# lipku/LiveTalking

Hardware: NVIDIA H100
Metric: lip-sync frames/sec (wav2lip256, 256x256, batch 16, mel + U-Net fwd + paste-back) (higher is better)
Workload: dtype f16 (fp32 accumulate); mel f64; paste u8

## Files before the change

### livetalking_b200/csrc/conv_halo.cu

```cuda
#include <cuda.h>

#include <atomic>
#include <mutex>
#include <utility>

#include "conv_halo.h"
#include "ltb_internal.h"
#include "ptx_sm90.cuh"

#ifdef LTB_HALO_DIAG
#include <cstdlib>
#define LTB_DIAG(bit) (p.dbg & (bit))
#else
#define LTB_DIAG(bit) 0
#endif

namespace ltb {

constexpr int kHaloP = 10;
constexpr int kHaloThreads = 384;
constexpr int kProducerRegs = 40, kConsumerRegs = 232;
constexpr int kSms = 132;

template <int BN, int NSUB, int NACC, int TAPS, int RC = 0>
struct HaloCfg {
  static constexpr bool HALO = (TAPS != 1);
  static constexpr bool S2 = (TAPS == 10);
  static constexpr int P = S2 ? 9 : (HALO ? kHaloP : 8);
  static constexpr int HR = S2 ? 16 * NSUB + 1 : (HALO ? 16 * NSUB + 2 : 16 * NSUB);
  static constexpr int TG = (TAPS == 9 || TAPS == 10) ? 3 : (TAPS == 16 ? 4 : 1);
  static constexpr int PLANE_BYTES = (HR * P * 128 + 1023) & ~1023;
  static constexpr int A_BYTES_RAW = (S2 ? 4 : 1) * HR * P * 128;
  static constexpr int A_BYTES = S2 ? 4 * PLANE_BYTES : ((A_BYTES_RAW + 1023) & ~1023);
  static constexpr int B_BYTES = TG * BN * 128;
  static constexpr int BUDGET = 223 * 1024;
  static constexpr int A_STAGES_STREAM = S2 ? 2 : ((BN <= 32) ? 4 : (BN <= 64 ? 3 : (NSUB == 1 ? 3 : 2)));
  static constexpr int A_STAGES_RES = ((BUDGET - RC * TG * B_BYTES) / A_BYTES) > 4 ? 4 : ((BUDGET - RC * TG * B_BYTES) / A_BYTES);
  static constexpr int A_STAGES = RC ? A_STAGES_RES : A_STAGES_STREAM;
  static constexpr bool RES_PREFETCH = (BN == 128 && NSUB == 2 && NACC == 1 && TAPS == 9 && RC == 0);
  static constexpr int RES_BYTES = RES_PREFETCH ? 128 * BN * 2 : 0;
  static constexpr int B_STAGES_MAX = (BUDGET - A_STAGES * A_BYTES - RES_BYTES) / B_BYTES;
  static constexpr int B_STAGES = RC ? RC * TG : (B_STAGES_MAX > 8 ? 8 : B_STAGES_MAX);
  static constexpr bool LAG = RC || B_STAGES >= 2 * TG;
  static constexpr int ACOLS = NACC * BN;
  static constexpr int SMEM_BYTES = A_STAGES * A_BYTES + B_STAGES * B_BYTES + RES_BYTES + 1024;
  static_assert(NSUB * ACOLS <= 256, "register accumulator overflow");
  static_assert(B_STAGES >= 2, "not enough shared memory for the weight ring");
  static_assert(A_STAGES >= 2, "not enough shared memory for the halo ring");
  static_assert(SMEM_BYTES + 3584 <= 227 * 1024, "shared memory overflow (dynamic + static)");
};

struct SubpixelView {
  int stage, view, slot0, brow, nslots;
};
constexpr int subpixel_view(int vy, int vx) { return (vy + 1) * kHaloP + (vx + 1); }
template <int TAPS>
struct SubpixelTable;
template <>
struct SubpixelTable<9> {
  static constexpr int NV = 5;
  static constexpr SubpixelView v[NV] = {{0, 0, 0, 0, 3}, {1, 1, 1, 0, 2}, {1, kHaloP + 1, 2, 2, 1}, {2, 0, 3, 2, 1}, {2, kHaloP, 2, 0, 2}};
};
template <>
struct SubpixelTable<16> {
  static constexpr int NV = 10;
  static constexpr SubpixelView v[NV] = {{0, subpixel_view(0, 0), 0, 0, 4},
                                         {1, subpixel_view(-1, 0), 0, 0, 2},  {1, subpixel_view(0, 1), 1, 2, 2},
                                         {2, subpixel_view(1, 0), 2, 0, 2},   {2, subpixel_view(0, -1), 0, 2, 1}, {2, subpixel_view(0, -1), 3, 3, 1},
                                         {3, subpixel_view(-1, -1), 0, 0, 1}, {3, subpixel_view(-1, 1), 1, 1, 1}, {3, subpixel_view(1, 1), 2, 2, 1},
                                         {3, subpixel_view(1, -1), 3, 3, 1}};
};

template <int BN, int SLOT0, int BROW, int R, size_t... S>
__device__ __forceinline__ void subpixel_slots(float (&acc)[R], uint64_t a, uint32_t b_lo, uint32_t b_hi, std::index_sequence<S...>) {
  (wgmma_ss_at<BN, (SLOT0 + (int)S) * BN>(acc, a, wgmma_lohi(b_lo + (BROW + (uint32_t)S) * BN * 8u, b_hi), 1u), ...);
}

template <int BN, int TAPS, int R, size_t... V>
__device__ __forceinline__ void subpixel_issue(float (&acc)[R], int j, int k, uint32_t a_lo0, uint32_t b_lo0, uint32_t a_hi, uint32_t b_hi,
                                               std::index_sequence<V...>) {
  (
      [&] {
        constexpr SubpixelView g = SubpixelTable<TAPS>::v[V];
        if (j == g.stage)
          subpixel_slots<BN, g.slot0, g.brow>(acc, wgmma_lohi(a_lo0 + g.view * 8u + k * 2u, a_hi), b_lo0 + k * 2u, b_hi,
                                              std::make_index_sequence<g.nslots>{});
      }(),
      ...);
}

__device__ __forceinline__ void quad_transpose(uint32_t (&x)[4], int lane) {
  const bool b2 = lane & 2, b1 = lane & 1;
  uint32_t s0 = __shfl_xor_sync(0xffffffffu, b2 ? x[0] : x[2], 2);
  uint32_t s1 = __shfl_xor_sync(0xffffffffu, b2 ? x[1] : x[3], 2);
  x[0] = b2 ? s0 : x[0];
  x[1] = b2 ? s1 : x[1];
  x[2] = b2 ? x[2] : s0;
  x[3] = b2 ? x[3] : s1;
  s0 = __shfl_xor_sync(0xffffffffu, b1 ? x[0] : x[1], 1);
  s1 = __shfl_xor_sync(0xffffffffu, b1 ? x[2] : x[3], 1);
  x[0] = b1 ? s0 : x[0];
  x[2] = b1 ? s1 : x[2];
  x[1] = b1 ? x[1] : s0;
  x[3] = b1 ? x[3] : s1;
}

constexpr bool halo_res_smem_ok(int BN, int NSUB, int NACC, int TAPS) { return TAPS == 9 && NACC == 1 && BN * NSUB <= 128; }

template <int BN, int NSUB, int NACC, int TAPS, int RC, bool GRP>
__global__ void __launch_bounds__(kHaloThreads, 1) conv_halo_wgmma_kernel(const __grid_constant__ HaloParams p) {
  static_assert(!GRP || TAPS == 1, "grouped weights exist in GEMM mode only");
  using C = HaloCfg<BN, NSUB, NACC, TAPS, RC>;
  extern __shared__ uint8_t smem_raw[];
  __shared__ __align__(8) uint64_t a_full[C::A_STAGES], a_empty[C::A_STAGES];
  __shared__ __align__(8) uint64_t b_full[C::B_STAGES], b_empty[C::B_STAGES];
  __shared__ float head_sw[100];
  constexpr int kGnSmem = (NACC == 1) ? 512 : 1;
  __shared__ float gn_acc[kGnSmem];

  const int tid = threadIdx.x, warp = tid >> 5, lane = tid & 31;
  constexpr bool kHeadOk = (BN == 32 && NACC == 1 && TAPS == 9);
  const bool gn_smem = NACC == 1 && p.gn_stats != nullptr && p.gn_images * p.gn_groups * 2 <= kGnSmem;
  if (gn_smem)
    for (int i = tid; i < p.gn_images * p.gn_groups * 2; i += kHaloThreads) gn_acc[i] = 0.f;
  constexpr bool kHaloMode = C::HALO;
  if (kHeadOk && p.head_out && tid < 99) head_sw[tid] = (tid < 96) ? p.head_w[tid] : p.head_b[tid - 96];
  const uint32_t smem0 = (smem_u32(smem_raw) + 1023u) & ~1023u;
  const uint32_t a_smem = smem0;
  const uint32_t b_smem = smem0 + C::A_STAGES * C::A_BYTES;
  const int chunks = (p.Cin + 63) / 64;
  const int kl_last = (p.Cin - 64 * (chunks - 1) + 15) / 16;

  if (tid == 0) {
    for (int s = 0; s < C::A_STAGES; ++s) {
      mbar_init(smem_u32(&a_full[s]), 1);
      mbar_init(smem_u32(&a_empty[s]), 8);
    }
    for (int s = 0; s < C::B_STAGES; ++s) {
      mbar_init(smem_u32(&b_full[s]), 1);
      mbar_init(smem_u32(&b_empty[s]), 8);
    }
    mbar_fence_init();
    tma_prefetch_desc(&p.tm_in);
    tma_prefetch_desc(&p.tm_w);
  }
  __syncthreads();

  const int tiles_m = kHaloMode ? p.tiles_x * p.tiles_y * p.N : p.tiles_x;

  pdl_launch_dependents();
  if (RC && warp == 8 && lane == 0) {
    mbar_arrive_expect_tx(smem_u32(&b_full[0]), RC * C::TG * C::B_BYTES);
    for (int c = 0; c < RC; ++c)
      for (int j = 0; j < C::TG; ++j)
        tma_load_3d(b_smem + (c * C::TG + j) * C::B_BYTES, &p.tm_w, smem_u32(&b_full[0]), c * 64, 0, j * C::TG);
  }
  pdl_wait();

// ... 744 lines not shown
```

### livetalking_b200/csrc/conv_plan.cu

```cuda
#include <cstring>
#include <string>
#include <vector>

#include "../../include/ltb200.h"
#include "conv_plan.h"
#include "ltb_internal.h"

namespace ltb {

static const int kTd[2][2] = {{0, 0}, {0, 1}};
static const int kTk[2][2] = {{1, 0}, {2, 0}};
static const int kTn[2] = {1, 2};
static const int kUd[2][2] = {{-1, 0}, {0, 1}};

ConvParams conv_params(ConvMode mode, int N, ConvSlice in, int IH, int IW, int Cin, ConvSlice out, int OH, int OW, int Cout,
                       ConvSlice res, const __half* w, int Ktot, int w_koff, const float* bias, bool relu, ConvTaps taps) {
  ConvParams p;
  std::memset(&p, 0, sizeof(p));
  p.in = in.p;
  p.N = N;
  p.IH = IH;
  p.IW = IW;
  p.ICtot = in.Ctot;
  p.ic_off = in.off;
// ... 10 lines not shown
  p.RCtot = res.Ctot;
  p.rc_off = res.off;
  p.w = w;
  p.Ktot = Ktot;
  p.bias = bias;
  p.relu = relu ? 1 : 0;
  if (mode == ConvMode::Dense) {
    p.sy = taps.sy;
    p.sx = taps.sx;
    p.GH = OH;
    p.GW = OW;
    p.nphases = 1;
    ConvPhase& ph = p.ph[0];
    ph.ntaps = taps.KH * taps.KW;
    ph.koff = w_koff;
    for (int kh = 0; kh < taps.KH; ++kh)
      for (int kw = 0; kw < taps.KW; ++kw) {
        ph.dy[kh * taps.KW + kw] = (signed char)(kh - taps.pad_t);
        ph.dx[kh * taps.KW + kw] = (signed char)(kw - taps.pad_l);
      }
  } else {
    const bool up = mode == ConvMode::Upsample2x;
    p.GH = IH;
    p.GW = IW;
    p.osy = p.osx = 2;
    p.nphases = 4;
    p.upconv = up ? 1 : 0;
    int koff = w_koff;
    for (int a = 0; a < 2; ++a)
      for (int b = 0; b < 2; ++b) {
        ConvPhase& ph = p.ph[a * 2 + b];
        const int na = up ? 2 : kTn[a], nb = up ? 2 : kTn[b];
        ph.ntaps = na * nb;
        ph.koff = koff;
        ph.ooy = a;
        ph.oox = b;
        for (int i = 0; i < na; ++i)
          for (int j = 0; j < nb; ++j) {
            ph.dy[i * nb + j] = (signed char)(up ? kUd[a][i] : kTd[a][i]);
            ph.dx[i * nb + j] = (signed char)(up ? kUd[b][j] : kTd[b][j]);
          }
        koff += ph.ntaps * Cin;
      }
  }
  p.M = N * p.GH * p.GW;
  return p;
}

int conv_plan(const ConvParams& p, const __half* w_tap, ConvPath path, ConvPlan* out) {
  out->p = p;
  out->halo = false;
  out->pingpong = false;
  out->rowpair = false;
  if (p.group_slot) {
    if (p.group_images < 1 || p.N % p.group_images || p.slots < 1 || p.w_slot_stride < 0 || p.bias_slot_stride < 0)
      return LTB_FAIL("conv: grouped weights need N divisible by group_images >= 1, slots >= 1 and non-negative slot strides");
    if (p.zbatch > 1 || p.upconv) return LTB_FAIL("conv: grouped weights cannot be combined with zbatch or the fused upsample");
  }
  if (path == ConvPath::Gather) return 0;
  if (w_tap && conv_pingpong_supported(p)) {
    if (conv_pingpong_make_plan(p, w_tap, &out->pp) != 0) return LTB_FAIL("conv: ping-pong plan / tensor map creation failed");
    out->pingpong = true;
    return 0;
  }
  if (w_tap && conv_rowpair_supported(p)) {
    if (conv_rowpair_make_plan(p, w_tap, &out->rp) != 0) return LTB_FAIL("conv: row-pair plan / tensor map creation failed");
    out->rowpair = true;
    return 0;
  }
  const bool gemm = p.nphases == 1 && p.ph[0].ntaps == 1;
  if (!((w_tap || gemm) && conv_halo_supported(p))) {
    if (path == ConvPath::Auto) return 0;
    return LTB_FAIL("conv: the halo kernel cannot run " + std::to_string(p.N) + "x" + std::to_string(p.IH) + "x" + std::to_string(p.IW) +
                    "x" + std::to_string(p.Cin) + " -> " + std::to_string(p.OH) + "x" + std::to_string(p.OW) + "x" + std::to_string(p.Cout) +
                    (w_tap || gemm ? "" : " without tap-major weights"));
  }
  if (conv_halo_make_plan(p, w_tap, &out->hp) != 0) return LTB_FAIL("conv: halo plan / tensor map creation failed");
  out->halo = true;
  return 0;
}

cudaError_t conv_launch(const ConvPlan& pl, cudaStream_t st, float* splitk_ws, size_t ws_floats) {
  if (pl.pingpong) return launch_conv_pingpong(pl.pp, st);
  if (pl.rowpair) return launch_conv_rowpair(pl.rp, st);
  return pl.halo ? launch_conv_halo(pl.hp, st) : launch_conv_gather(pl.p, st, splitk_ws, ws_floats);
}

bool conv_plan_variant(const ConvPlan& pl, bool have_ws, size_t ws_floats, ltb_conv_variant* out) {
  std::memset(out, 0, sizeof(*out));
  out->grouped = pl.p.group_slot != nullptr;
  if (pl.pingpong) {
    out->kernel = 2;
    out->taps = 9;
    out->bn = 64;
    out->nsub = 1;
    out->nacc = 1;
    out->resident_chunks = 1;
    out->res_halo = 1;
    return true;
  }
  if (pl.rowpair) {
    out->kernel = 3;
    out->taps = 9;
    out->bn = 32;
    out->nsub = 1;
    out->nacc = 1;
    out->resident_chunks = 2;
    return true;
  }
  if (pl.halo) {
    out->kernel = 1;
    out->taps = pl.hp.TAPS;
    out->bn = pl.hp.BN;
    out->nsub = pl.hp.NSUB;
    out->nacc = pl.hp.NACC;
    out->resident_chunks = conv_halo_resident_chunks(pl.hp, conv_halo_sms());
    out->res_halo = pl.hp.hp.res_halo;
    return true;
  }
  int ksplit = 0;
  if (!conv_gather_pick(pl.p, have_ws, ws_floats, &out->bn, &out->kb, &ksplit)) return false;
  out->ksplit = ksplit > 1 ? ksplit : 1;
  return true;
}

bool conv_plan_fuse_gn_stats(ConvPlan* pl, float* stats, int groups, int hw) {
  const ConvParams& p = pl->p;
  if (!pl->halo || pl->hp.grouped || p.oc_off != 0 || p.OCtot != p.Cout || !conv_halo_gn_fusable(pl->hp, p.Cout, groups, hw)) return false;
  HaloParams& h = pl->hp.hp;
  h.gn_stats = stats;
  h.gn_groups = groups;
  h.gn_cpg = p.Cout / groups;
  h.gn_hw = hw;
  h.gn_images = p.M / hw;
  return true;
}

bool conv_plan_fuse_head(ConvPlan* pl, const float* w, const float* b, float* out) {
  if (pl->rowpair) {
    pl->rp.head_w = w;
    pl->rp.head_b = b;
    pl->rp.head_out = out;
    return true;
  }
  if (!pl->halo || pl->hp.grouped || pl->hp.BN != 32 || pl->p.Cout != 32) return false;
  pl->hp.hp.head_w = w;
  pl->hp.hp.head_b = b;
  pl->hp.hp.head_out = out;
  return true;
}

static void pack_conv_w(const float* w, int cout, int cin, int KH, int KW, std::vector<__half>& out) {
  out.resize((size_t)cout * KH * KW * cin);
  for (int co = 0; co < cout; ++co)
    for (int kh = 0; kh < KH; ++kh)
      for (int kw = 0; kw < KW; ++kw)
        for (int ci = 0; ci < cin; ++ci)
          out[((size_t)co * KH * KW + kh * KW + kw) * cin + ci] = __float2half(w[(((size_t)co * cin + ci) * KH + kh) * KW + kw]);
}
static void pack_convT_w(const float* w, int cin, int cout, std::vector<__half>& out) {
// ... 36 lines not shown
  }
  if (OH <= 0 || OW <= 0) return LTB_FAIL("empty output");
  const size_t in_b = (size_t)d->N * d->IH * d->IW * d->Cin * 2, out_b = (size_t)d->N * OH * OW * d->Cout * 2;
  __half *din = nullptr, *dout = nullptr, *dw = nullptr, *dres = nullptr, *dwt = nullptr;
  float* dbias = nullptr;
  float* dws = nullptr;
  cudaEvent_t e0 = nullptr, e1 = nullptr;
  int rc = 0;
  auto cleanup = [&]() {
    cudaFree(din);
    cudaFree(dout);
    cudaFree(dw);
    cudaFree(dres);
    cudaFree(dwt);
    cudaFree(dws);
    cudaFree(dbias);
    if (e0) cudaEventDestroy(e0);
    if (e1) cudaEventDestroy(e1);
  };
#define CK(x)                                                             \
  do {                                                                    \
    cudaError_t _e = (x);                                                 \
    if (_e != cudaSuccess) {                                              \
      rc = LTB_FAIL(std::string(#x) + ": " + cudaGetErrorString(_e));     \
      cleanup();                                                          \
      return rc;                                                          \
    }                                                                     \
  } while (0)
  CK(cudaMalloc(&din, in_b));
  CK(cudaMalloc(&dout, out_b));
  CK(cudaMalloc(&dw, wp.size() * 2));
  CK(cudaMalloc(&dbias, (size_t)d->Cout * 4));
  CK(cudaMemcpy(din, in_f16, in_b, cudaMemcpyHostToDevice));
  CK(cudaMemcpy(dw, wp.data(), wp.size() * 2, cudaMemcpyHostToDevice));
  CK(cudaMemcpy(dbias, bias_f32, (size_t)d->Cout * 4, cudaMemcpyHostToDevice));
  CK(cudaMemset(dout, 0xFF, out_b));
  if (d->has_res) {
    CK(cudaMalloc(&dres, out_b));
    CK(cudaMemcpy(dres, res_f16, out_b, cudaMemcpyHostToDevice));
  }
  if (d->KH == 3 && d->KW == 3) {
    CK(cudaMalloc(&dwt, wp.size() * 2));
    CK(d->transposed ? launch_w_tap_major_convT(dw, dwt, d->Cout, d->Cin, nullptr) : launch_w_tap_major(dw, dwt, d->Cout, d->Cin, nullptr));
  }
  const ConvParams p = conv_params(d->transposed ? ConvMode::Transposed : ConvMode::Dense, d->N, {din, d->Cin, 0}, d->IH, d->IW, d->Cin,
                                   {dout, d->Cout, 0}, OH, OW, d->Cout, d->has_res ? ConvSlice{dres, d->Cout, 0} : ConvSlice{}, dw, Ktot, 0,
                                   dbias, d->relu != 0, {d->KH, d->KW, d->sy, d->sx, d->pad, d->pad});
  const ConvPath path = d->force_path == 1 ? ConvPath::Gather : d->force_path == 2 ? ConvPath::Halo : ConvPath::Auto;
  ConvPlan pl;
  if (conv_plan(p, dwt, path, &pl)) {
    cleanup();
    return 1;
  }
  const size_t ws_floats = (pl.halo || pl.pingpong || pl.rowpair) ? 0 : (size_t)1 << 22;
  if (ws_floats) {
    CK(cudaMalloc(&dws, ws_floats * sizeof(float)));
    CK(cudaMemset(dws, 0, ws_floats * sizeof(float)));
  }
  CK(conv_launch(pl, nullptr, dws, ws_floats));
  if (reps > 0) {
    CK(cudaEventCreate(&e0));
    CK(cudaEventCreate(&e1));
    for (int i = 0; i < 3; ++i) CK(conv_launch(pl, nullptr, dws, ws_floats));
    CK(cudaEventRecord(e0, nullptr));
    for (int i = 0; i < reps; ++i) CK(conv_launch(pl, nullptr, dws, ws_floats));
    CK(cudaEventRecord(e1, nullptr));
    CK(cudaEventSynchronize(e1));
    CK(cudaEventElapsedTime(ms_out, e0, e1));
    *ms_out /= reps;
  }
  CK(cudaDeviceSynchronize());
  CK(cudaMemcpy(out_f16, dout, out_b, cudaMemcpyDeviceToHost));
#undef CK
  cleanup();
  return 0;
}

extern "C" {

int ltb_conv2d_f16(const ltb_conv_desc* d, const void* in_f16, const float* w_f32, const float* bias_f32,
                   const void* res_f16, void* out_f16) {
  return conv2d_f16_impl(d, in_f16, w_f32, bias_f32, res_f16, out_f16, 0, nullptr);
}

int ltb_conv2d_f16_timed(const ltb_conv_desc* d, const void* in_f16, const float* w_f32, const float* bias_f32,
                         const void* res_f16, void* out_f16, int reps, float* ms_per_launch) {
  if (reps < 1 || !ms_per_launch) return LTB_FAIL("conv2d_f16_timed: reps >= 1 and a result pointer are required");
  return conv2d_f16_impl(d, in_f16, w_f32, bias_f32, res_f16, out_f16, reps, ms_per_launch);
}

}
```

### livetalking_b200/csrc/conv_plan.h

```cpp
#pragma once
#include <cuda_runtime.h>

#include "conv_halo.h"
#include "conv_pingpong.h"
#include "conv_rowpair.h"

struct ltb_conv_variant;

namespace ltb {

struct ConvSlice {
  const __half* p;
  int Ctot, off;
};

enum class ConvMode {
  Dense,
  Transposed,
  Upsample2x,
};
struct ConvTaps {
  int KH, KW, sy, sx, pad_t, pad_l;
};

inline int conv_out_dim(int in, int k, int s, int pad) { return (in + 2 * pad - k) / s + 1; }

ConvParams conv_params(ConvMode mode, int N, ConvSlice in, int IH, int IW, int Cin, ConvSlice out, int OH, int OW, int Cout,
                       ConvSlice res, const __half* w, int Ktot, int w_koff, const float* bias, bool relu, ConvTaps taps = {});

enum class ConvPath {
  Auto,
  Gather,
  Halo,
};
struct ConvPlan {
  ConvParams p{};
  bool halo = false;
  HaloPlan hp{};
  bool pingpong = false;
  PingpongParams pp{};
  bool rowpair = false;
  RowpairParams rp{};
};

int conv_plan(const ConvParams& p, const __half* w_tap, ConvPath path, ConvPlan* out);
cudaError_t conv_launch(const ConvPlan& pl, cudaStream_t st, float* splitk_ws, size_t ws_floats);
bool conv_plan_variant(const ConvPlan& pl, bool have_ws, size_t ws_floats, ltb_conv_variant* out);

bool conv_plan_fuse_gn_stats(ConvPlan* pl, float* stats, int groups, int hw);
bool conv_plan_fuse_head(ConvPlan* pl, const float* w, const float* b, float* out);

}
```

### livetalking_b200/csrc/ltb_internal.h

```cpp
#pragma once
#include <cuda_runtime.h>
#include <cuda_fp16.h>
#include <cstdint>
#include <cstdio>
#include <atomic>
#include <cstdlib>
#include <utility>
#include <string>

#include "conv_params.h"

namespace ltb {

void set_error(const std::string& msg);
int fail(const char* file, int line, const std::string& msg);
#define LTB_FAIL(msg) ::ltb::fail(__FILE__, __LINE__, (msg))
#define LTB_CUDA(expr)                                                                         \
  do {                                                                                         \
    cudaError_t _e = (expr);                                                                   \
    if (_e != cudaSuccess) {                                                                   \
      cudaGetLastError();  \
      return LTB_FAIL(std::string(#expr) + ": " + cudaGetErrorString(_e));                     \
    }                                                                                          \
  } while (0)

struct SmemConfigOnce {
  std::atomic<unsigned long long> done{0};
  template <typename K>
  cudaError_t ensure(K kernel, int bytes) {
    int dev = 0;
    cudaError_t e = cudaGetDevice(&dev);
    if (e != cudaSuccess) return e;
    const unsigned long long bit = 1ull << (dev & 63);
    if (done.load(std::memory_order_acquire) & bit) return cudaSuccess;
    e = cudaFuncSetAttribute(kernel, cudaFuncAttributeMaxDynamicSharedMemorySize, bytes);
    if (e == cudaSuccess) done.fetch_or(bit, std::memory_order_release);
    return e;
  }
};

bool pdl_default();
bool pdl_enabled();
void pdl_set_enabled(bool on);

template <typename... KArgs, typename... Args>
inline cudaError_t launch_kernel_pdl(void (*kernel)(KArgs...), dim3 grid, dim3 block, size_t smem, cudaStream_t st, Args&&... args) {
  cudaLaunchConfig_t cfg = {};
  cfg.gridDim = grid;
  cfg.blockDim = block;
  cfg.dynamicSmemBytes = smem;
  cfg.stream = st;
  cudaLaunchAttribute attr[1];
  attr[0].id = cudaLaunchAttributeProgrammaticStreamSerialization;
  attr[0].val.programmaticStreamSerializationAllowed = 1;
  cfg.attrs = attr;
  cfg.numAttrs = pdl_enabled() ? 1 : 0;
  return cudaLaunchKernelEx(&cfg, kernel, std::forward<Args>(args)...);
}

template <typename... KArgs, typename... Args>
inline cudaError_t launch_kernel_plain(void (*kernel)(KArgs...), dim3 grid, dim3 block, size_t smem, cudaStream_t st, Args&&... args) {
  cudaLaunchConfig_t cfg = {};
  cfg.gridDim = grid;
  cfg.blockDim = block;
  cfg.dynamicSmemBytes = smem;
  cfg.stream = st;
  cfg.numAttrs = 0;
  return cudaLaunchKernelEx(&cfg, kernel, std::forward<Args>(args)...);
}

struct SlotDesc {
  const uint8_t* face;
  const uint8_t* frame;
  int y1, y2, x1, x2;
};

cudaError_t launch_conv_gather(const ConvParams& p, cudaStream_t st, float* splitk_ws = nullptr, size_t splitk_ws_floats = 0);
bool conv_gather_pick(const ConvParams& p, bool have_ws, size_t splitk_ws_floats, int* bn, int* kb, int* ksplit);

cudaError_t launch_w2l_prep_faces(const uint8_t* faces, int nfaces, const int* d_index, int B, __half* img_pad, cudaStream_t st,
                                  const SlotDesc* slots = nullptr);
cudaError_t launch_set_int(int* p, int v, cudaStream_t st);
cudaError_t launch_w2l_audio_conv0(const float* mel, const float* w9x32, const float* bias, __half* out, int B, cudaStream_t st);
cudaError_t launch_w2l_head(const __half* x, const float* w3x32, const float* b3, float* pred, int npix, cudaStream_t st);

cudaError_t launch_mel_step(const float* pcm, int nsamp, int B, int stride_left_chunks, int fps, double* scratch_spec,
                            double* scratch_mel, float* out, cudaStream_t st);
size_t mel_scratch_spec_doubles(int nsamp);
size_t mel_scratch_mel_doubles(int nsamp);

cudaError_t launch_w2l_paste(const uint8_t* frames, const int* coords, int nf, int H, int W, const float* pred, int slot0,
                             int index, int explicit_idx, int count, uint8_t* out, cudaStream_t st, const SlotDesc* slots = nullptr);

}
```

### livetalking_b200/csrc/ptx_sm90.cuh

```cuda
#pragma once
#include <cuda_fp16.h>
#include <cstdint>
#include <cstdio>

namespace ltb {

__device__ __forceinline__ uint32_t smem_u32(const void* p) {
  return static_cast<uint32_t>(__cvta_generic_to_shared(p));
}

__device__ __forceinline__ void mbar_init(uint32_t bar, uint32_t count) {
  asm volatile("mbarrier.init.shared::cta.b64 [%0], %1;" ::"r"(bar), "r"(count) : "memory");
}
__device__ __forceinline__ void mbar_fence_init() {
  asm volatile("fence.mbarrier_init.release.cluster;" ::: "memory");
}
__device__ __forceinline__ void mbar_arrive(uint32_t bar) {
  asm volatile("mbarrier.arrive.shared::cta.b64 _, [%0];" ::"r"(bar) : "memory");
}
__device__ __forceinline__ void mbar_arrive_expect_tx(uint32_t bar, uint32_t bytes) {
  asm volatile("mbarrier.arrive.expect_tx.shared::cta.b64 _, [%0], %1;" ::"r"(bar), "r"(bytes) : "memory");
}
__device__ __forceinline__ bool mbar_try_wait(uint32_t bar, uint32_t parity) {
  uint32_t ok;
// ... 10 lines not shown
  if (mbar_try_wait(bar, parity)) return;
  const long long t0 = clock64();
  while (!mbar_try_wait(bar, parity)) {
    if (clock64() - t0 > 8000000000LL) __trap();
  }
}

__device__ __forceinline__ void fence_proxy_async_smem() {
  asm volatile("fence.proxy.async.shared::cta;" ::: "memory");
}

__device__ __forceinline__ void cp_async16(uint32_t dst, const void* src, uint32_t src_bytes) {
  asm volatile("cp.async.cg.shared.global [%0], [%1], 16, %2;" ::"r"(dst), "l"(src), "r"(src_bytes) : "memory");
}
__device__ __forceinline__ void cp_async_commit() { asm volatile("cp.async.commit_group;" ::: "memory"); }
template <int N>
__device__ __forceinline__ void cp_async_wait() {
  asm volatile("cp.async.wait_group %0;" ::"n"(N) : "memory");
}
__device__ __forceinline__ uint4 lds128(uint32_t addr) {
  uint4 v;
  asm volatile("ld.shared.v4.u32 {%0, %1, %2, %3}, [%4];" : "=r"(v.x), "=r"(v.y), "=r"(v.z), "=r"(v.w) : "r"(addr) : "memory");
  return v;
}

__device__ __forceinline__ void tma_prefetch_desc(const void* tmap) {
  asm volatile("prefetch.tensormap [%0];" ::"l"(tmap) : "memory");
}
__device__ __forceinline__ void tma_load_2d(uint32_t dst, const void* tmap, uint32_t bar, int c0, int c1) {
  asm volatile(
      "cp.async.bulk.tensor.2d.shared::cluster.global.mbarrier::complete_tx::bytes [%0], [%1, {%3, %4}], [%2];" ::"r"(dst),
      "l"(tmap), "r"(bar), "r"(c0), "r"(c1)
      : "memory");
}
__device__ __forceinline__ void tma_load_3d(uint32_t dst, const void* tmap, uint32_t bar, int c0, int c1, int c2) {
  asm volatile(
      "cp.async.bulk.tensor.3d.shared::cluster.global.mbarrier::complete_tx::bytes [%0], [%1, {%3, %4, %5}], [%2];" ::"r"(dst),
      "l"(tmap), "r"(bar), "r"(c0), "r"(c1), "r"(c2)
      : "memory");
}
__device__ __forceinline__ void tma_load_4d(uint32_t dst, const void* tmap, uint32_t bar, int c0, int c1, int c2, int c3) {
  asm volatile(
      "cp.async.bulk.tensor.4d.shared::cluster.global.mbarrier::complete_tx::bytes [%0], [%1, {%3, %4, %5, %6}], [%2];" ::"r"(
          dst),
      "l"(tmap), "r"(bar), "r"(c0), "r"(c1), "r"(c2), "r"(c3)
      : "memory");
}
__device__ __forceinline__ void tma_load_5d(uint32_t dst, const void* tmap, uint32_t bar, int c0, int c1, int c2, int c3,
                                            int c4) {
  asm volatile(
      "cp.async.bulk.tensor.5d.shared::cluster.global.mbarrier::complete_tx::bytes [%0], [%1, {%3, %4, %5, %6, %7}], [%2];" ::
          "r"(dst),
      "l"(tmap), "r"(bar), "r"(c0), "r"(c1), "r"(c2), "r"(c3), "r"(c4)
      : "memory");
}

__device__ __forceinline__ void ldmatrix_x4(uint32_t& r0, uint32_t& r1, uint32_t& r2, uint32_t& r3, uint32_t saddr) {
  asm volatile("ldmatrix.sync.aligned.m8n8.x4.shared.b16 {%0, %1, %2, %3}, [%4];"
               : "=r"(r0), "=r"(r1), "=r"(r2), "=r"(r3)
               : "r"(saddr)
               : "memory");
}

__device__ __forceinline__ void ldmatrix_x4_trans(uint32_t& r0, uint32_t& r1, uint32_t& r2, uint32_t& r3, uint32_t saddr) {
  asm volatile("ldmatrix.sync.aligned.m8n8.x4.trans.shared.b16 {%0, %1, %2, %3}, [%4];"
               : "=r"(r0), "=r"(r1), "=r"(r2), "=r"(r3)
               : "r"(saddr)
               : "memory");
}
__device__ __forceinline__ void stmatrix_x4_trans(uint32_t saddr, uint32_t r0, uint32_t r1, uint32_t r2, uint32_t r3) {
  asm volatile("stmatrix.sync.aligned.m8n8.x4.trans.shared.b16 [%0], {%1, %2, %3, %4};" ::"r"(saddr), "r"(r0), "r"(r1), "r"(r2), "r"(r3)
               : "memory");
}

__device__ __forceinline__ void tma_store_4d(const void* tmap, uint32_t src, int c0, int c1, int c2, int c3) {
  asm volatile("cp.async.bulk.tensor.4d.global.shared::cta.bulk_group [%0, {%2, %3, %4, %5}], [%1];" ::"l"(tmap), "r"(src), "r"(c0),
               "r"(c1), "r"(c2), "r"(c3)
               : "memory");
}
__device__ __forceinline__ void bulk_commit() { asm volatile("cp.async.bulk.commit_group;" ::: "memory"); }
template <int N>
__device__ __forceinline__ void bulk_wait_read() {
  asm volatile("cp.async.bulk.wait_group.read %0;" ::"n"(N) : "memory");
}
template <int N>
__device__ __forceinline__ void bulk_wait() {
  asm volatile("cp.async.bulk.wait_group %0;" ::"n"(N) : "memory");
}

__device__ __forceinline__ void named_sync(uint32_t id, uint32_t threads) {
  asm volatile("bar.sync %0, %1;" ::"r"(id), "r"(threads) : "memory");
}
__device__ __forceinline__ void named_arrive(uint32_t id, uint32_t threads) {
  asm volatile("bar.arrive %0, %1;" ::"r"(id), "r"(threads) : "memory");
}

__device__ __forceinline__ uint64_t wgmma_desc(uint32_t saddr, uint32_t lbo_bytes, uint32_t sbo_bytes, uint32_t layout) {
  uint64_t d = 0;
  d |= (uint64_t)((saddr & 0x3FFFF) >> 4);
  d |= (uint64_t)((lbo_bytes >> 4) & 0x3FFF) << 16;
  d |= (uint64_t)((sbo_bytes >> 4) & 0x3FFF) << 32;
  d |= (uint64_t)(layout & 3) << 62;
  return d;
}
__host__ __device__ constexpr uint32_t wgmma_hi_128b(uint32_t sbo_bytes) { return (sbo_bytes >> 4) | (1u << 30); }
__host__ __device__ constexpr uint32_t wgmma_hi_32b(uint32_t sbo_bytes) { return (sbo_bytes >> 4) | (3u << 30); }
// ... 204 lines not shown
```

### livetalking_b200/csrc/w2l_engine.cu

```cuda
#include <cstring>
#include <memory>
#include <mutex>
#include <string>
#include <vector>

#include "../../include/ltb200.h"
#include "conv_plan.h"
#include "ltb_internal.h"
#include "stem_umma.h"

namespace ltb {

static thread_local std::string g_last_error;
void set_error(const std::string& msg) { g_last_error = msg; }

bool pdl_default() {
  static const bool on = [] {
    const char* e = std::getenv("LTB_NO_PDL");
    return !(e && e[0] && e[0] != '0');
  }();
  return on;
}
static thread_local int g_pdl = -1;
bool pdl_enabled() { return g_pdl < 0 ? pdl_default() : g_pdl == 1; }
// ... 240 lines not shown
  const int catS[8] = {512, 512, 512, 256, 128, 64, 32, 16};
  __half* cat[8];
  for (int i = 0; i < 8; ++i) {
    void* p;
    if (dev_alloc(s, (size_t)B * catH[i] * catH[i] * (catD[i] + catS[i]) * 2, &p, true)) return 1;
    cat[i] = static_cast<__half*>(p);
  }
  const size_t tmp_bytes = (size_t)B * 256 * 256 * 64 * 2;
  __half* ring[2] = {nullptr, nullptr};
  int ring_next = 0;
  auto new_tmp = [&](int H, int W, int C, View* v) -> int {
    void* p = nullptr;
    if (keep) {
      if (dev_alloc(s, (size_t)B * H * W * C * 2, &p, true)) return 1;
    } else {
      if (!ring[ring_next]) {
        if (dev_alloc(s, tmp_bytes, &p, true)) return 1;
        ring[ring_next] = static_cast<__half*>(p);
      }
      p = ring[ring_next];
      ring_next ^= 1;
    }
    *v = View{static_cast<__half*>(p), H, W, C, 0, C};
    return 0;
  };
  __half* aring[2] = {nullptr, nullptr};
  int aring_next = 0;
  auto new_atmp = [&](int H, int W, int C, View* v) -> int {
    void* p = nullptr;
    if (keep) {
      if (dev_alloc(s, (size_t)B * H * W * C * 2, &p, true)) return 1;
    } else {
      if (!aring[aring_next]) {
        if (dev_alloc(s, (size_t)B * 80 * 16 * 32 * 2, &p, true)) return 1;
        aring[aring_next] = static_cast<__half*>(p);
      }
      p = aring[aring_next];
      aring_next ^= 1;
    }
    *v = View{static_cast<__half*>(p), H, W, C, 0, C};
    return 0;
  };
  auto cat_dec = [&](int i) { return View{cat[i], catH[i], catH[i], catD[i] + catS[i], 0, catD[i]}; };
  auto cat_skip = [&](int i) { return View{cat[i], catH[i], catH[i], catD[i] + catS[i], catD[i], catS[i]}; };
  auto cat_all = [&](int i) { return View{cat[i], catH[i], catH[i], catD[i] + catS[i], 0, catD[i] + catS[i]}; };

  auto record = [&](int li, const View& v) {
    s->louts[li] = LayerOut{v.p, v.H, v.W, v.C, v.Ctot, v.c_off};
  };
  const ConvPath path = (s->flags & LTB_SESSION_NO_HALO) ? ConvPath::Gather : ConvPath::Auto;
  auto push_conv = [&](int li, const ConvParams& p) -> int {
    Op o;
    if (conv_plan(p, m->wt[li], path, &o.conv)) return LTB_FAIL("plan: layer " + std::to_string(li) + ": " + g_last_error);
    o.type = (o.conv.halo || o.conv.pingpong || o.conv.rowpair) ? 4 : 0;
    s->ops.push_back(o);
    return 0;
  };
  auto add_conv = [&](int li, const View& in, const View& out, const View* res) -> int {
    const LDef& L = kLayers[li];
    if (in.C != L.cin || out.C != L.cout) return LTB_FAIL("plan: channel mismatch at layer " + std::to_string(li));
    const int OH = conv_out_dim(in.H, L.k, L.sy, L.pad), OW = conv_out_dim(in.W, L.k, L.sx, L.pad);
    if (OH != out.H || OW != out.W) return LTB_FAIL("plan: spatial mismatch at layer " + std::to_string(li));
    const ConvParams p = conv_params(ConvMode::Dense, B, in.slice(), in.H, in.W, L.cin, out.slice(), OH, OW, L.cout,
                                     res ? res->slice() : ConvSlice{}, m->w[li], L.k * L.k * L.cin, 0, m->bias[li], true,
                                     {L.k, L.k, L.sy, L.sx, L.pad, L.pad});
    if (push_conv(li, p)) return 1;
    record(li, out);
    return 0;
  };
  auto add_convT = [&](int li, const View& in, const View& out) -> int {
    const LDef& L = kLayers[li];
    if (in.C != L.cin || out.C != L.cout || out.H != 2 * in.H) return LTB_FAIL("plan: convT mismatch at layer " + std::to_string(li));
    const ConvParams p = conv_params(ConvMode::Transposed, B, in.slice(), in.H, in.W, L.cin, out.slice(), out.H, out.W, L.cout,
                                     ConvSlice{}, m->w[li], 9 * L.cin, 0, m->bias[li], true);
    if (push_conv(li, p)) return 1;
    record(li, out);
    return 0;
  };

  {
    Op o;
    o.type = 6;
    o.branch = 1;
    s->ops.push_back(o);
  }
  View a_prev;
  if (new_atmp(80, 16, 32, &a_prev)) return 1;
  {
    Op o;
    o.type = 2;
    o.audio_out = a_prev.p;
    o.branch = 1;
    s->ops.push_back(o);
    record(0, a_prev);
  }
  {
    int H = 80, W = 16;
    for (int li = 1; li <= 12; ++li) {
      const LDef& L = kLayers[li];
      const int OH = conv_out_dim(H, L.k, L.sy, L.pad), OW = conv_out_dim(W, L.k, L.sx, L.pad);
      View o;
      if (new_atmp(OH, OW, L.cout, &o)) return 1;
      if (add_conv(li, a_prev, o, L.res ? &a_prev : nullptr)) return 1;
      s->ops.back().branch = 1;
      a_prev = o;
      H = OH;
      W = OW;
// ... 750 lines not shown
```

Before: 7386.

## Add 2-CTA cluster sub-pixel conv kernel with multicast weight loads

Adds a new cluster-of-two kernel for 3x3 sub-pixel (NACC=4, BN=64) halo convolutions. Each CTA in the pair loads half of each weight tile and multicasts it to both, so weight traffic per CTA is halved while each CTA keeps its own input halo. Empty barriers are released across the cluster. It is selected automatically for eligible large non-residual layers, at the cost of cluster scheduling constraints and cross-CTA synchronisation.

New measurement: 7441, median of 6. No clear change (+0.8%).

```diff
diff --git a/livetalking_b200/csrc/conv_halo.cu b/livetalking_b200/csrc/conv_halo.cu
--- a/livetalking_b200/csrc/conv_halo.cu
+++ b/livetalking_b200/csrc/conv_halo.cu
@@ -5,6 +5,7 @@
 #include <utility>
 
 #include "conv_halo.h"
+#include "conv_subpixel.cuh"
 #include "ltb_internal.h"
 #include "ptx_sm90.cuh"
 
@@ -17,7 +18,6 @@
 
 namespace ltb {
 
-constexpr int kHaloP = 10;
 constexpr int kHaloThreads = 384;
 constexpr int kProducerRegs = 40, kConsumerRegs = 232;
 constexpr int kSms = 132;
@@ -49,61 +49,6 @@
   static_assert(A_STAGES >= 2, "not enough shared memory for the halo ring");
   static_assert(SMEM_BYTES + 3584 <= 227 * 1024, "shared memory overflow (dynamic + static)");
 };
-
-struct SubpixelView {
-  int stage, view, slot0, brow, nslots;
-};
-constexpr int subpixel_view(int vy, int vx) { return (vy + 1) * kHaloP + (vx + 1); }
-template <int TAPS>
-struct SubpixelTable;
-template <>
-struct SubpixelTable<9> {
-  static constexpr int NV = 5;
-  static constexpr SubpixelView v[NV] = {{0, 0, 0, 0, 3}, {1, 1, 1, 0, 2}, {1, kHaloP + 1, 2, 2, 1}, {2, 0, 3, 2, 1}, {2, kHaloP, 2, 0, 2}};
-};
-template <>
-struct SubpixelTable<16> {
-  static constexpr int NV = 10;
-  static constexpr SubpixelView v[NV] = {{0, subpixel_view(0, 0), 0, 0, 4},
-                                         {1, subpixel_view(-1, 0), 0, 0, 2},  {1, subpixel_view(0, 1), 1, 2, 2},
-                                         {2, subpixel_view(1, 0), 2, 0, 2},   {2, subpixel_view(0, -1), 0, 2, 1}, {2, subpixel_view(0, -1), 3, 3, 1},
-                                         {3, subpixel_view(-1, -1), 0, 0, 1}, {3, subpixel_view(-1, 1), 1, 1, 1}, {3, subpixel_view(1, 1), 2, 2, 1},
-                                         {3, subpixel_view(1, -1), 3, 3, 1}};
-};
-
-template <int BN, int SLOT0, int BROW, int R, size_t... S>
-__device__ __forceinline__ void subpixel_slots(float (&acc)[R], uint64_t a, uint32_t b_lo, uint32_t b_hi, std::index_sequence<S...>) {
-  (wgmma_ss_at<BN, (SLOT0 + (int)S) * BN>(acc, a, wgmma_lohi(b_lo + (BROW + (uint32_t)S) * BN * 8u, b_hi), 1u), ...);
-}
-
-template <int BN, int TAPS, int R, size_t... V>
-__device__ __forceinline__ void subpixel_issue(float (&acc)[R], int j, int k, uint32_t a_lo0, uint32_t b_lo0, uint32_t a_hi, uint32_t b_hi,
-                                               std::index_sequence<V...>) {
-  (
-      [&] {
-        constexpr SubpixelView g = SubpixelTable<TAPS>::v[V];
-        if (j == g.stage)
-          subpixel_slots<BN, g.slot0, g.brow>(acc, wgmma_lohi(a_lo0 + g.view * 8u + k * 2u, a_hi), b_lo0 + k * 2u, b_hi,
-                                              std::make_index_sequence<g.nslots>{});
-      }(),
-      ...);
-}
-
-__device__ __forceinline__ void quad_transpose(uint32_t (&x)[4], int lane) {
-  const bool b2 = lane & 2, b1 = lane & 1;
-  uint32_t s0 = __shfl_xor_sync(0xffffffffu, b2 ? x[0] : x[2], 2);
-  uint32_t s1 = __shfl_xor_sync(0xffffffffu, b2 ? x[1] : x[3], 2);
-  x[0] = b2 ? s0 : x[0];
-  x[1] = b2 ? s1 : x[1];
-  x[2] = b2 ? x[2] : s0;
-  x[3] = b2 ? x[3] : s1;
-  s0 = __shfl_xor_sync(0xffffffffu, b1 ? x[0] : x[1], 1);
-  s1 = __shfl_xor_sync(0xffffffffu, b1 ? x[2] : x[3], 1);
-  x[0] = b1 ? s0 : x[0];
-  x[2] = b1 ? s1 : x[2];
-  x[1] = b1 ? x[1] : s0;
-  x[3] = b1 ? x[3] : s1;
-}
 
 constexpr bool halo_res_smem_ok(int BN, int NSUB, int NACC, int TAPS) { return TAPS == 9 && NACC == 1 && BN * NSUB <= 128; }
 
diff --git a/livetalking_b200/csrc/conv_plan.cu b/livetalking_b200/csrc/conv_plan.cu
--- a/livetalking_b200/csrc/conv_plan.cu
+++ b/livetalking_b200/csrc/conv_plan.cu
@@ -86,6 +86,7 @@
   out->halo = false;
   out->pingpong = false;
   out->rowpair = false;
+  out->pair = false;
   if (p.group_slot) {
     if (p.group_images < 1 || p.N % p.group_images || p.slots < 1 || p.w_slot_stride < 0 || p.bias_slot_stride < 0)
       return LTB_FAIL("conv: grouped weights need N divisible by group_images >= 1, slots >= 1 and non-negative slot strides");
@@ -110,6 +111,11 @@
                     (w_tap || gemm ? "" : " without tap-major weights"));
   }
   if (conv_halo_make_plan(p, w_tap, &out->hp) != 0) return LTB_FAIL("conv: halo plan / tensor map creation failed");
+  if (conv_subpixel_pair_supported(p, out->hp)) {
+    if (conv_subpixel_pair_make_plan(p, w_tap, &out->hp) != 0) return LTB_FAIL("conv: sub-pixel pair plan / tensor map creation failed");
+    out->pair = true;
+    return 0;
+  }
   out->halo = true;
   return 0;
 }
@@ -117,6 +123,7 @@
 cudaError_t conv_launch(const ConvPlan& pl, cudaStream_t st, float* splitk_ws, size_t ws_floats) {
   if (pl.pingpong) return launch_conv_pingpong(pl.pp, st);
   if (pl.rowpair) return launch_conv_rowpair(pl.rp, st);
+  if (pl.pair) return launch_conv_subpixel_pair(pl.hp, st);
   return pl.halo ? launch_conv_halo(pl.hp, st) : launch_conv_gather(pl.p, st, splitk_ws, ws_floats);
 }
 
@@ -140,6 +147,14 @@
     out->nsub = 1;
     out->nacc = 1;
     out->resident_chunks = 2;
+    return true;
+  }
+  if (pl.pair) {
+    out->kernel = 4;
+    out->taps = 9;
+    out->bn = 64;
+    out->nsub = 1;
+    out->nacc = 4;
     return true;
   }
   if (pl.halo) {
@@ -282,7 +297,7 @@
     cleanup();
     return 1;
   }
-  const size_t ws_floats = (pl.halo || pl.pingpong || pl.rowpair) ? 0 : (size_t)1 << 22;
+  const size_t ws_floats = (pl.halo || pl.pingpong || pl.rowpair || pl.pair) ? 0 : (size_t)1 << 22;
   if (ws_floats) {
     CK(cudaMalloc(&dws, ws_floats * sizeof(float)));
     CK(cudaMemset(dws, 0, ws_floats * sizeof(float)));
diff --git a/livetalking_b200/csrc/conv_plan.h b/livetalking_b200/csrc/conv_plan.h
--- a/livetalking_b200/csrc/conv_plan.h
+++ b/livetalking_b200/csrc/conv_plan.h
@@ -4,6 +4,7 @@
 #include "conv_halo.h"
 #include "conv_pingpong.h"
 #include "conv_rowpair.h"
+#include "conv_subpixel_pair.h"
 
 struct ltb_conv_variant;
 
@@ -41,6 +42,7 @@
   PingpongParams pp{};
   bool rowpair = false;
   RowpairParams rp{};
+  bool pair = false;
 };
 
 int conv_plan(const ConvParams& p, const __half* w_tap, ConvPath path, ConvPlan* out);
diff --git a/livetalking_b200/csrc/conv_subpixel.cuh b/livetalking_b200/csrc/conv_subpixel.cuh
--- /dev/null
+++ b/livetalking_b200/csrc/conv_subpixel.cuh
@@ -0,0 +1,66 @@
+#pragma once
+#include <cstdint>
+#include <utility>
+
+#include "ptx_sm90.cuh"
+
+namespace ltb {
+
+constexpr int kHaloP = 10;
+
+struct SubpixelView {
+  int stage, view, slot0, brow, nslots;
+};
+constexpr int subpixel_view(int vy, int vx) { return (vy + 1) * kHaloP + (vx + 1); }
+template <int TAPS>
+struct SubpixelTable;
+template <>
+struct SubpixelTable<9> {
+  static constexpr int NV = 5;
+  static constexpr SubpixelView v[NV] = {{0, 0, 0, 0, 3}, {1, 1, 1, 0, 2}, {1, kHaloP + 1, 2, 2, 1}, {2, 0, 3, 2, 1}, {2, kHaloP, 2, 0, 2}};
+};
+template <>
+struct SubpixelTable<16> {
+  static constexpr int NV = 10;
+  static constexpr SubpixelView v[NV] = {{0, subpixel_view(0, 0), 0, 0, 4},
+                                         {1, subpixel_view(-1, 0), 0, 0, 2},  {1, subpixel_view(0, 1), 1, 2, 2},
+                                         {2, subpixel_view(1, 0), 2, 0, 2},   {2, subpixel_view(0, -1), 0, 2, 1}, {2, subpixel_view(0, -1), 3, 3, 1},
+                                         {3, subpixel_view(-1, -1), 0, 0, 1}, {3, subpixel_view(-1, 1), 1, 1, 1}, {3, subpixel_view(1, 1), 2, 2, 1},
+                                         {3, subpixel_view(1, -1), 3, 3, 1}};
+};
+
+template <int BN, int SLOT0, int BROW, int R, size_t... S>
+__device__ __forceinline__ void subpixel_slots(float (&acc)[R], uint64_t a, uint32_t b_lo, uint32_t b_hi, std::index_sequence<S...>) {
+  (wgmma_ss_at<BN, (SLOT0 + (int)S) * BN>(acc, a, wgmma_lohi(b_lo + (BROW + (uint32_t)S) * BN * 8u, b_hi), 1u), ...);
+}
+
+template <int BN, int TAPS, int R, size_t... V>
+__device__ __forceinline__ void subpixel_issue(float (&acc)[R], int j, int k, uint32_t a_lo0, uint32_t b_lo0, uint32_t a_hi, uint32_t b_hi,
+                                               std::index_sequence<V...>) {
+  (
+      [&] {
+        constexpr SubpixelView g = SubpixelTable<TAPS>::v[V];
+        if (j == g.stage)
+          subpixel_slots<BN, g.slot0, g.brow>(acc, wgmma_lohi(a_lo0 + g.view * 8u + k * 2u, a_hi), b_lo0 + k * 2u, b_hi,
+                                              std::make_index_sequence<g.nslots>{});
+      }(),
+      ...);
+}
+
+__device__ __forceinline__ void quad_transpose(uint32_t (&x)[4], int lane) {
+  const bool b2 = lane & 2, b1 = lane & 1;
+  uint32_t s0 = __shfl_xor_sync(0xffffffffu, b2 ? x[0] : x[2], 2);
+  uint32_t s1 = __shfl_xor_sync(0xffffffffu, b2 ? x[1] : x[3], 2);
+  x[0] = b2 ? s0 : x[0];
+  x[1] = b2 ? s1 : x[1];
+  x[2] = b2 ? x[2] : s0;
+  x[3] = b2 ? x[3] : s1;
+  s0 = __shfl_xor_sync(0xffffffffu, b1 ? x[0] : x[1], 1);
+  s1 = __shfl_xor_sync(0xffffffffu, b1 ? x[2] : x[3], 1);
+  x[0] = b1 ? s0 : x[0];
+  x[2] = b1 ? s1 : x[2];
+  x[1] = b1 ? x[1] : s0;
+  x[3] = b1 ? x[3] : s1;
+}
+
+}
diff --git a/livetalking_b200/csrc/conv_subpixel_pair.cu b/livetalking_b200/csrc/conv_subpixel_pair.cu
--- /dev/null
+++ b/livetalking_b200/csrc/conv_subpixel_pair.cu
@@ -0,0 +1,255 @@
+#include <cuda.h>
+
+#include <atomic>
+#include <cstdlib>
+#include <cstring>
+
+#include "conv_subpixel.cuh"
+#include "conv_subpixel_pair.h"
+#include "ltb_internal.h"
+#include "ptx_sm90.cuh"
+
+namespace ltb {
+
+namespace {
+
+constexpr int kThreads = 384;
+constexpr int kProducerRegs = 40, kConsumerRegs = 232;
+constexpr int kBN = 64;
+constexpr int kABytesRaw = 18 * kHaloP * 128;
+constexpr int kABytes = (kABytesRaw + 1023) & ~1023;
+constexpr int kAStages = 3;
+constexpr int kTG = 3;
+constexpr int kSlice = kBN * 128;
+constexpr int kHalf = kSlice / 2;
+constexpr int kBBytes = kTG * kSlice;
+constexpr int kBStages = 6;
+constexpr int kSmemBytes = kAStages * kABytes + kBStages * kBBytes + 1024;
+static_assert(kSmemBytes + 1024 <= 227 * 1024, "shared memory overflow");
+
+}
+
+__global__ void __launch_bounds__(kThreads, 1) conv_subpixel_pair_kernel(const __grid_constant__ HaloParams p) {
+  extern __shared__ uint8_t smem_raw[];
+  __shared__ __align__(8) uint64_t a_full[kAStages], a_empty[kAStages];
+  __shared__ __align__(8) uint64_t b_full[kBStages], b_empty[kBStages];
+  const int tid = threadIdx.x, warp = tid >> 5, lane = tid & 31;
+  const uint32_t rank = cluster_ctarank();
+  const uint32_t smem0 = (smem_u32(smem_raw) + 1023u) & ~1023u;
+  const uint32_t a_smem = smem0;
+  const uint32_t b_smem = smem0 + kAStages * kABytes;
+  const int chunks = (p.Cin + 63) / 64;
+  const int kl_last = (p.Cin - 64 * (chunks - 1) + 15) / 16;
+
+  if (tid == 0) {
+    for (int s = 0; s < kAStages; ++s) {
+      mbar_init(smem_u32(&a_full[s]), 1);
+      mbar_init(smem_u32(&a_empty[s]), 8);
+    }
+    for (int s = 0; s < kBStages; ++s) {
+      mbar_init(smem_u32(&b_full[s]), 1);
+      mbar_init(smem_u32(&b_empty[s]), 16);
+    }
+    mbar_fence_init();
+    tma_prefetch_desc(&p.tm_in);
+    tma_prefetch_desc(&p.tm_w);
+  }
+  cluster_sync();
+
+  const int tiles_img = p.tiles_x * p.tiles_y;
+  const int pairs_m = (tiles_img * p.N + 1) / 2;
+  const int total_pairs = pairs_m * p.tiles_n;
+  const int cluster = blockIdx.x >> 1, nclusters = gridDim.x >> 1;
+  auto tile_of = [&](int q, int& nt, int& img, int& ty, int& tx) {
+    nt = q / pairs_m;
+    int mt = 2 * (q - nt * pairs_m) + (int)rank;
+    img = mt / tiles_img;
+    mt -= img * tiles_img;
+    ty = mt / p.tiles_x;
+    tx = mt - ty * p.tiles_x;
+  };
+
+  pdl_launch_dependents();
+  pdl_wait();
+
+  if (warp >= 8) {
+    setmaxnreg_dec<kProducerRegs>();
+    if (warp == 8 && lane == 0) {
+      uint32_t ai = 0, bi = 0;
+      for (int q = cluster; q < total_pairs; q += nclusters) {
+        int nt, img, ty, tx;
+        tile_of(q, nt, img, ty, tx);
+        for (int c = 0; c < chunks; ++c) {
+          const uint32_t as = ai % kAStages;
+          mbar_wait(smem_u32(&a_empty[as]), ((ai / kAStages) & 1u) ^ 1u);
+          mbar_arrive_expect_tx(smem_u32(&a_full[as]), kABytesRaw);
+          tma_load_4d(a_smem + as * kABytes, &p.tm_in, smem_u32(&a_full[as]), c * 64, tx * 8 + p.halo_x0, ty * 16 + p.halo_y0, img);
+          ++ai;
+          for (int j = 0; j < kTG; ++j) {
+            const uint32_t bs = bi % kBStages;
+            mbar_wait(smem_u32(&b_empty[bs]), ((bi / kBStages) & 1u) ^ 1u);
+            mbar_arrive_expect_tx(smem_u32(&b_full[bs]), kBBytes);
+            for (int t = 0; t < kTG; ++t)
+              tma_load_3d_multicast(b_smem + bs * kBBytes + t * kSlice + rank * kHalf, &p.tm_w, smem_u32(&b_full[bs]), c * 64,
+                                    nt * kBN + 32 * (int)rank, j * kTG + t, 0x3);
+            ++bi;
+          }
+        }
+      }
+    }
+  } else {
+    setmaxnreg_inc<kConsumerRegs>();
+    const int wg = warp >> 2, wq = warp & 3;
+    const int cq = 2 * (lane & 3);
+    constexpr uint32_t kAHi = wgmma_hi_128b(kHaloP * 128);
+    constexpr uint32_t kBHi = wgmma_hi_128b(1024);
+    const uint32_t wg_off = (uint32_t)wg * 8u * kHaloP * 8u;
+    auto release_b = [&](uint32_t bs) {
+      mbar_arrive(smem_u32(&b_empty[bs]));
+      mbar_arrive_cluster(mapa_shared(smem_u32(&b_empty[bs]), rank ^ 1u));
+    };
+    uint32_t ai = 0, bi = 0;
+    for (int q = cluster; q < total_pairs; q += nclusters) {
+      int nt, img, ty, tx;
+      tile_of(q, nt, img, ty, tx);
+      const int n0 = nt * kBN;
+      float acc[2 * kBN];
+#pragma unroll
+      for (int i = 0; i < 2 * kBN; ++i) acc[i] = 0.f;
+      uint32_t pend_as = 0, pend_bs = 0;
+      bool pend = false;
+      auto run_chunk = [&](auto kl_t) {
+        constexpr int KL = decltype(kl_t)::value;
+        const uint32_t as = ai % kAStages;
+        mbar_wait(smem_u32(&a_full[as]), (ai / kAStages) & 1u);
+        const uint32_t a_lo0 = wgmma_lo(a_smem + as * kABytes) + wg_off;
+        const uint32_t bs0 = bi % kBStages;
+#pragma unroll
+        for (int j = 0; j < kTG; ++j) {
+          const uint32_t bs = (bi + j) % kBStages;
+          mbar_wait(smem_u32(&b_full[bs]), ((bi + j) / kBStages) & 1u);
+          const uint32_t b_lo0 = wgmma_lo(b_smem + bs * kBBytes);
+          wgmma_fence();
+#pragma unroll
+          for (int k = 0; k < KL; ++k)
+            subpixel_issue<kBN, 9>(acc, j, k, a_lo0, b_lo0, kAHi, kBHi, std::make_index_sequence<SubpixelTable<9>::NV>{});
+        }
+        wgmma_commit();
+        wgmma_wait<1>();
+        if (pend) {
+          __syncwarp();
+          if (lane == 0) {
+            mbar_arrive(smem_u32(&a_empty[pend_as]));
+            for (int j = 0; j < kTG; ++j) release_b((pend_bs + j) % kBStages);
+          }
+        }
+        pend = true;
+        pend_as = as;
+        pend_bs = bs0;
+        ++ai;
+        bi += kTG;
+      };
+      const bool ragged = kl_last <= 2;
+#pragma unroll 1
+      for (int c = 0; c < chunks - ragged; ++c) run_chunk(std::integral_constant<int, 4>{});
+      if (ragged) run_chunk(std::integral_constant<int, 2>{});
+      wgmma_wait<0>();
+      wgmma_fence_regs(acc);
+      __syncwarp();
+      if (lane == 0) {
+        mbar_arrive(smem_u32(&a_empty[pend_as]));
+        for (int j = 0; j < kTG; ++j) release_b((pend_bs + j) % kBStages);
+      }
+
+      float2 bb[kBN / 8];
+#pragma unroll
+      for (int i = 0; i < kBN / 8; ++i) bb[i] = __ldg(reinterpret_cast<const float2*>(p.bias + n0 + 8 * i + cq));
+      const bool row_ok = img < p.N;
+#pragma unroll
+      for (int sl = 0; sl < 4; ++sl) {
+#pragma unroll
+        for (int hh = 0; hh < 2; ++hh) {
+          const int r = wq * 16 + (lane >> 2) + 8 * hh;
+          const int gy = ty * 16 + wg * 8 + (r >> 3), gx = tx * 8 + (r & 7);
+          const size_t opix = ((size_t)img * p.OH + gy * p.osy + p.acc_oy[sl]) * p.OW + gx * p.osx + p.acc_ox[sl];
+          uint4* optr = reinterpret_cast<uint4*>(p.out + opix * p.OCtot + p.oc_off + n0 + 8 * (lane & 3));
+#pragma unroll
+          for (int m = 0; m < kBN / 32; ++m) {
+            uint32_t v[4];
+#pragma unroll
+            for (int j = 0; j < 4; ++j) {
+              const int i = 4 * m + j;
+              const float f0 = acc[sl * kBN / 2 + 4 * i + 2 * hh] + bb[i].x;
+              const float f1 = acc[sl * kBN / 2 + 4 * i + 2 * hh + 1] + bb[i].y;
+              v[j] = p.relu ? f32x2_to_f16x2_sat_relu(f0, f1) : f32x2_to_f16x2_sat(f0, f1);
+            }
+            quad_transpose(v, lane);
+            if (row_ok) optr[4 * m] = make_uint4(v[0], v[1], v[2], v[3]);
+          }
+        }
+      }
+    }
+  }
+
+  __syncwarp();
+  cluster_sync();
+}
+
+static SmemConfigOnce g_smem_once;
+
+static int pair_clusters() {
+  static std::atomic<int> cached{0};
+  int n = cached.load();
+  if (n) return n;
+  if (g_smem_once.ensure(conv_subpixel_pair_kernel, kSmemBytes) != cudaSuccess) return 0;
+  cudaLaunchConfig_t cfg = {};
+  cfg.gridDim = dim3(2 * conv_halo_sms());
+  cfg.blockDim = dim3(kThreads);
+  cfg.dynamicSmemBytes = kSmemBytes;
+  cudaLaunchAttribute attr[1];
+  attr[0].id = cudaLaunchAttributeClusterDimension;
+  attr[0].val.clusterDim.x = 2;
+  attr[0].val.clusterDim.y = 1;
+  attr[0].val.clusterDim.z = 1;
+  cfg.attrs = attr;
+  cfg.numAttrs = 1;
+  if (cudaOccupancyMaxActiveClusters(&n, conv_subpixel_pair_kernel, &cfg) != cudaSuccess || n <= 0) {
+    cudaGetLastError();
+    return 0;
+  }
+  cached.store(n);
+  return n;
+}
+
+static bool pair_enabled() {
+  const char* e = std::getenv("LTB_CONV_PAIR");
+  return !(e && std::strcmp(e, "0") == 0);
+}
+
+bool conv_subpixel_pair_supported(const ConvParams& p, const HaloPlan& hp) {
+  if (hp.TAPS != 9 || hp.NACC != 4 || p.upconv || hp.BN != kBN || hp.NSUB != 1 || hp.grouped) return false;
+  if (p.Cin < 128 || p.res || p.GH % 16 || p.GW % 8) return false;
+  const int sms = conv_halo_sms();
+  if (conv_halo_resident_chunks(hp, sms) != 0 || hp.hp.total_tiles < 8 * sms) return false;
+  return pair_enabled() && pair_clusters() > 0;
+}
+
+int conv_subpixel_pair_make_plan(const ConvParams& p, const __half* w_tap_major, HaloPlan* hp) {
+  if (!conv_subpixel_pair_supported(p, *hp) || !w_tap_major) return 1;
+  const cuuint64_t dims[3] = {(cuuint64_t)p.Cin, (cuuint64_t)p.Cout, 9};
+  const cuuint64_t strides[2] = {(cuuint64_t)p.Cin * 2, (cuuint64_t)p.Cout * p.Cin * 2};
+  const cuuint32_t box[3] = {64, 32, 1};
+  return encode_tmap_f16(&hp->hp.tm_w, 3, w_tap_major, dims, strides, box) ? 0 : 2;
+}
+
+cudaError_t launch_conv_subpixel_pair(const HaloPlan& pl, cudaStream_t st) {
+  if (cudaError_t e = g_smem_once.ensure(conv_subpixel_pair_kernel, kSmemBytes); e != cudaSuccess) return e;
+  const int clusters = pair_clusters();
+  if (clusters <= 0) return cudaErrorInvalidConfiguration;
+  const HaloParams& h = pl.hp;
+  const int pairs = (h.tiles_x * h.tiles_y * h.N + 1) / 2 * h.tiles_n;
+  const int grid = 2 * (pairs < clusters ? pairs : clusters);
+  return launch_kernel_pdl_cluster(conv_subpixel_pair_kernel, dim3(grid), dim3(kThreads), dim3(2, 1, 1), kSmemBytes, st, h);
+}
+
+}
diff --git a/livetalking_b200/csrc/conv_subpixel_pair.h b/livetalking_b200/csrc/conv_subpixel_pair.h
--- /dev/null
+++ b/livetalking_b200/csrc/conv_subpixel_pair.h
@@ -0,0 +1,12 @@
+#pragma once
+#include <cuda_runtime.h>
+
+#include "conv_halo.h"
+
+namespace ltb {
+
+bool conv_subpixel_pair_supported(const ConvParams& p, const HaloPlan& hp);
+int conv_subpixel_pair_make_plan(const ConvParams& p, const __half* w_tap_major, HaloPlan* hp);
+cudaError_t launch_conv_subpixel_pair(const HaloPlan& pl, cudaStream_t st);
+
+}
diff --git a/livetalking_b200/csrc/ltb_internal.h b/livetalking_b200/csrc/ltb_internal.h
--- a/livetalking_b200/csrc/ltb_internal.h
+++ b/livetalking_b200/csrc/ltb_internal.h
@@ -59,6 +59,26 @@
 }
 
 template <typename... KArgs, typename... Args>
+inline cudaError_t launch_kernel_pdl_cluster(void (*kernel)(KArgs...), dim3 grid, dim3 block, dim3 cluster, size_t smem, cudaStream_t st,
+                                             Args&&... args) {
+  cudaLaunchConfig_t cfg = {};
+  cfg.gridDim = grid;
+  cfg.blockDim = block;
+  cfg.dynamicSmemBytes = smem;
+  cfg.stream = st;
+  cudaLaunchAttribute attr[2];
+  attr[0].id = cudaLaunchAttributeClusterDimension;
+  attr[0].val.clusterDim.x = cluster.x;
+  attr[0].val.clusterDim.y = cluster.y;
+  attr[0].val.clusterDim.z = cluster.z;
+  attr[1].id = cudaLaunchAttributeProgrammaticStreamSerialization;
+  attr[1].val.programmaticStreamSerializationAllowed = 1;
+  cfg.attrs = attr;
+  cfg.numAttrs = pdl_enabled() ? 2 : 1;
+  return cudaLaunchKernelEx(&cfg, kernel, std::forward<Args>(args)...);
+}
+
+template <typename... KArgs, typename... Args>
 inline cudaError_t launch_kernel_plain(void (*kernel)(KArgs...), dim3 grid, dim3 block, size_t smem, cudaStream_t st, Args&&... args) {
   cudaLaunchConfig_t cfg = {};
   cfg.gridDim = grid;
diff --git a/livetalking_b200/csrc/ptx_sm90.cuh b/livetalking_b200/csrc/ptx_sm90.cuh
--- a/livetalking_b200/csrc/ptx_sm90.cuh
+++ b/livetalking_b200/csrc/ptx_sm90.cuh
@@ -86,6 +86,29 @@
       "cp.async.bulk.tensor.5d.shared::cluster.global.mbarrier::complete_tx::bytes [%0], [%1, {%3, %4, %5, %6, %7}], [%2];" ::
           "r"(dst),
       "l"(tmap), "r"(bar), "r"(c0), "r"(c1), "r"(c2), "r"(c3), "r"(c4)
+      : "memory");
+}
+
+__device__ __forceinline__ uint32_t cluster_ctarank() {
+  uint32_t r;
+  asm volatile("mov.u32 %0, %%cluster_ctarank;" : "=r"(r));
+  return r;
+}
+__device__ __forceinline__ uint32_t mapa_shared(uint32_t addr, uint32_t rank) {
+  uint32_t r;
+  asm volatile("mapa.shared::cluster.u32 %0, %1, %2;" : "=r"(r) : "r"(addr), "r"(rank));
+  return r;
+}
+__device__ __forceinline__ void mbar_arrive_cluster(uint32_t remote_bar) {
+  asm volatile("mbarrier.arrive.shared::cluster.b64 _, [%0];" ::"r"(remote_bar) : "memory");
+}
+__device__ __forceinline__ void cluster_sync() {
+  asm volatile("barrier.cluster.arrive.release.aligned;\n\tbarrier.cluster.wait.acquire.aligned;" ::: "memory");
+}
+__device__ __forceinline__ void tma_load_3d_multicast(uint32_t dst, const void* tmap, uint32_t bar, int c0, int c1, int c2, uint16_t cta_mask) {
+  asm volatile(
+      "cp.async.bulk.tensor.3d.shared::cluster.global.mbarrier::complete_tx::bytes.multicast::cluster [%0], [%1, {%3, %4, %5}], [%2], %6;" ::"r"(dst),
+      "l"(tmap), "r"(bar), "r"(c0), "r"(c1), "r"(c2), "h"(cta_mask)
       : "memory");
 }
 
diff --git a/livetalking_b200/csrc/w2l_engine.cu b/livetalking_b200/csrc/w2l_engine.cu
--- a/livetalking_b200/csrc/w2l_engine.cu
+++ b/livetalking_b200/csrc/w2l_engine.cu
@@ -316,7 +316,7 @@
   auto push_conv = [&](int li, const ConvParams& p) -> int {
     Op o;
     if (conv_plan(p, m->wt[li], path, &o.conv)) return LTB_FAIL("plan: layer " + std::to_string(li) + ": " + g_last_error);
-    o.type = (o.conv.halo || o.conv.pingpong || o.conv.rowpair) ? 4 : 0;
+    o.type = (o.conv.halo || o.conv.pingpong || o.conv.rowpair || o.conv.pair) ? 4 : 0;
     s->ops.push_back(o);
     return 0;
   };
```
